# qmoututu11/Image_Restoration_and_Enhancement

Measured on AMD Instinct MI355X. Metric: restored images/sec @512x512, 50 DDIM steps; PSNR/SSIM vs reference, higher is better.
Workload: dtype bf16; 1 GPU; BASELINE configs[1] denoise 512x512, batch 8/GPU, 50 DDIM steps x strength 0.5 = 25 UNet evals, CFG 5.0 (UNet batch 16); task=denoise, global_batch=8, resolution=512, compute=UNet + CLIP bf16, VAE fp16 (fp32 accumulation), parallelism=dp1, weights_bcast=none, outputs_finite=True

## Files before the change

### image_restoration_and_enhancement_amd/_lib.py

```python
from __future__ import annotations

import ctypes as C
import os
from pathlib import Path

_PKG = Path(__file__).resolve().parent
LIB_PATH = Path(os.environ.get("IRX_LIB", _PKG / "libirx.so"))

IRX_F32, IRX_BF16, IRX_F16 = 0, 1, 2
IRX_MODEL_UNET, IRX_MODEL_VAE, IRX_MODEL_CLIP = 0, 1, 2
IRX_MODEL_LPIPS = 3
IRX_MODEL_FID = 4
IRX_MODEL_SRVGG = 5
IRX_LAYOUT_VEC, IRX_LAYOUT_MAT, IRX_LAYOUT_CONV, IRX_LAYOUT_EMB = 0, 1, 2, 3
IRX_LAYOUT_MAT_GEGLU64, IRX_LAYOUT_VEC_GEGLU64 = 4, 5
IRX_LAYOUT_VEC_LN_U, IRX_LAYOUT_VEC_LN_V = 6, 7
IRX_LAYOUT_MAT_CHAIN, IRX_LAYOUT_VEC_CHAIN = 8, 9
IRX_LAYOUT_CONV_UP2 = 10
IRX_RCCL_ID_BYTES = 128
IRX_RESAMPLE_LANCZOS, IRX_RESAMPLE_BICUBIC, IRX_RESAMPLE_MAX_KSIZE = 0, 1, 97


class IrxError(RuntimeError):
    pass
# ... 134 lines not shown
    "irx_op_gn_conv3": (i32, [vp, i32, vp, vp, i32, i32, i32, i32, i32, i32, f32, vp, vp, i32, vp, vp, i32, vp, i64,
                              vp, vp, vp, vp]),
    "irx_op_gn_conv_narrow": (i32, [vp, i32, vp, i32, i32, i32, i32, i32, f32, vp, vp, i32, vp, vp, i32, vp, i32, i32,
                                    vp]),
    "irx_op_gn_proj_ws_bytes": (sz, [i32, i32, i32, i32, i32]),
    "irx_op_gn_proj": (i32, [vp, i32, vp, i32, i32, i32, i32, f32, vp, vp, vp, vp, i32, vp, vp, C.POINTER(i32),
                             C.POINTER(i32)]),
    "irx_op_layer_norm": (i32, [vp, i32, vp, i32, i32, f32, vp, vp, vp]),
    "irx_op_attention": (i32, [vp, i32, i32, i32, i32, i32, i32, vp, i64, i64, vp, i64, i64, vp, i64, i64, vp,
                               i64, i64, f32, i32]),
    "irx_op_attention_hm": (i32, [vp, i32, i32, i32, i32, i32, i32, vp, vp, vp, vp, f32]),
    "irx_op_geglu": (i32, [vp, i32, vp, i32, i32, vp]),
    "irx_op_gemm_geglu": (i32, [vp, i32, i32, i32, i32, vp, vp, vp, vp]),
    "irx_op_gemm_ln_out": (i32, [vp, i32, i32, i32, i32, vp, vp, vp, vp, vp, vp, i32, f32]),
    "irx_op_gemm_ln_fold": (i32, [vp, i32, i32, i32, i32, vp, vp, vp, vp, vp, vp, i32, i32, vp]),
    "irx_op_conv2d_gn_parts": (i32, [vp, i32, vp, vp, i32, i32, i32, i32, i32, i32, i32, vp, vp, i32, i32, i32, i32,
                                     i32, i32, i32, i32, vp, i64, vp, vp, i32, i32, vp, vp, C.POINTER(i32),
                                     C.POINTER(i32), C.POINTER(i32), C.POINTER(sz)]),
    "irx_op_gemm_gn_parts": (i32, [vp, i32, i32, i32, i32, vp, vp, vp, vp, i32, vp, vp, vp, C.POINTER(i32),
                                   C.POINTER(i32), C.POINTER(sz)]),
    "irx_op_upsample_conv_gn_parts": (i32, [vp, i32, vp, i32, i32, i32, i32, vp, vp, vp, vp, vp, C.POINTER(i32),
                                            C.POINTER(i32), C.POINTER(sz)]),
    "irx_op_group_norm_parts": (i32, [vp, i32, vp, vp, i32, i32, i32, i32, i32, f32, vp, vp, i32, vp, vp, i32, vp, i32,
                                      vp]),
    "irx_op_group_norm_parts_ab": (i32, [vp, i32, i32, i32, i32, f32, vp, vp, vp, i32, vp, vp]),
    "irx_op_softmax_rows": (i32, [vp, i32, vp, i64, i32, i32, vp, i64]),
    "irx_op_transpose2d": (i32, [vp, i32, vp, i64, i32, i32, vp, i64, i32, i64, i64]),
    "irx_op_timestep_embed": (i32, [vp, i32, vp, i32, i32, i32, f32, vp]),
    "irx_op_embed_tokens": (i32, [vp, i32, vp, i32, i32, vp, vp, i32, vp]),
}
# ... 89 lines not shown
```

### image_restoration_and_enhancement_amd/csrc/capi.cpp

```cpp
#include <algorithm>
#include <cmath>
#include <cstring>
#include <string>

#include "../../include/irx.h"
#include "gemm_plan.h"
#include "models.h"
#include "profile.h"

namespace irx {
static thread_local std::string g_err;
void set_error(const std::string& m) { g_err = m; }
const char* last_error() { return g_err.c_str(); }
extern int g_attn_pf80;
}

using namespace irx;

struct irx_model {
  std::unique_ptr<Model> m;
};

#define IRX_API_BEGIN try {
#define IRX_API_END                                       \
// ... 971 lines not shown

int irx_op_attention_hm(void* s, int dtype, int B, int H, int lq, int lk, int d, const void* q, const void* k,
                        const void* v, void* o, float scale) {
  IRX_API_BEGIN
  AttnArgs a;
  a.dtype = dtype; a.B = B; a.H = H; a.Lq = lq; a.Lk = lk; a.d = d;
  a.q = q; a.ldq = d; a.sq = (long)H * lq * d; a.hsq = (long)lq * d;
  a.k = k; a.ldk = d; a.sk = (long)H * lk * d; a.hsk = (long)lk * d;
  a.v = v; a.ldv = d; a.sv = (long)H * lk * d; a.hsv = (long)lk * d;
  a.o = o; a.ldo = d; a.so = (long)H * lq * d; a.hso = (long)lq * d;
  a.scale = scale;
  attention(a, S(s));
  IRX_API_END
}

int irx_op_gemm_ln_out(void* s, int dtype, int M, int N, int K, const void* A, const void* B, const float* bias,
                       const void* residual, void* C, void* parts, int final_rs, float eps) {
  IRX_API_BEGIN
  GemmArgs a;
  a.dtype = dtype; a.M = M; a.N = N; a.K = K;
  a.A = A; a.lda = K; a.B = B; a.ldb = K;
  a.C = C; a.ldc = N; a.bias = bias;
  a.residual = residual; a.ldr = N;
  a.imgs = g_op_imgs;
  a.ln_out_rs = final_rs;
  a.ln_eps = eps;
  IRX_CHECK(parts && gemm_emits_ln_parts(a), "shape/dtype cannot emit LayerNorm partials");
  a.ln_out = (float2*)parts;
  gemm(a, S(s));
  IRX_API_END
}

int irx_op_gemm_ln_fold(void* s, int dtype, int M, int N, int K, const void* A, const void* B, const float* u,
                        const float* v, const void* rs, const void* parts, int T, int geglu, void* C) {
  IRX_API_BEGIN
  IRX_CHECK((rs != nullptr) != (parts != nullptr), "give the row statistics or the partials, not both");
  GemmArgs a;
  a.dtype = dtype; a.M = M; a.N = N; a.K = K;
  a.A = A; a.lda = K; a.B = B; a.ldb = K;
  a.C = C; a.ldc = geglu ? N / 2 : N; a.bias = v; a.geglu = geglu ? 1 : 0;
  a.ln_u = u;
  a.ln_rs = (const float2*)rs;
  a.ln_part = (const float2*)parts;
  a.ln_T = parts ? T : 0;
  a.imgs = g_op_imgs;
  IRX_CHECK(!geglu || gemm_geglu_fusable(a), "shape/dtype not eligible for the fused GEGLU epilogue");
  IRX_CHECK(gemm_ln_foldable(a), "shape/dtype not eligible for the folded LayerNorm epilogue");
  gemm(a, S(s));
  IRX_API_END
}

int irx_op_gemm_geglu(void* s, int dtype, int M, int N, int K, const void* A, const void* B, const float* bias,
                      void* C) {
  IRX_API_BEGIN
  GemmArgs a;
  a.dtype = dtype; a.M = M; a.N = N; a.K = K;
  a.A = A; a.lda = K; a.B = B; a.ldb = K;
  a.C = C; a.ldc = N / 2; a.bias = bias; a.geglu = 1;
  a.imgs = g_op_imgs;
// ... 179 lines not shown
```

### image_restoration_and_enhancement_amd/csrc/gemm.hip

```cpp
#include "gemm_plan.h"
#include "profile.h"

namespace irx {

namespace {

constexpr int kThreads = 256;

struct RowInfo {
  int n;
  int iy0, ix0;
};

template <typename T, int WM, int WN, int TM, int TN, bool CONV, bool OUTF32, bool HS = false>
__global__ __launch_bounds__(kThreads, 2) void gemm_kernel(GemmArgs a) {
  constexpr int VEC = 16 / (int)sizeof(T);
  constexpr int BK = 8 * VEC;
  constexpr int BM = WM * TM * 16;
  constexpr int BN = WN * TN * 16;
  constexpr int AR = (BM * 8 + kThreads - 1) / kThreads;
  constexpr int BR = (BN * 8 + kThreads - 1) / kThreads;
  static_assert(WM * WN == 4, "4 waves");
  __shared__ uint4 smem[2][(BM + BN) * 8];

// ... 230 lines not shown
                                a.res_rows < a.M && a.M <= 2 * a.res_rows),
            "repeating residual (res_rows): 16-bit, batch 1, res_rows < M <= 2 res_rows");
  if (a.conv) {
    const ConvGeom& g = a.g;
    IRX_CHECK(g.src0 && g.C0 % vec == 0 && g.C1 % vec == 0, "conv channels must be 16-byte multiples");
    IRX_CHECK(((uintptr_t)g.src0 % 16) == 0 && (!g.src1 || ((uintptr_t)g.src1 % 16) == 0), "conv source alignment");
    IRX_CHECK(g.C1 == 0 || g.src1, "concat source missing");
    IRX_CHECK(a.K == g.KH * g.KW * (g.C0 + g.C1), "conv K mismatch");
    IRX_CHECK(a.M == g.N * g.Ho * g.Wo, "conv M mismatch");
    IRX_CHECK(g.Hv >= g.Hin && g.Wv >= g.Win, "virtual (upsampled) size must not shrink");
  } else {
    IRX_CHECK(a.A && a.lda % vec == 0 && ((uintptr_t)a.A % 16) == 0, "A rows must be 16-byte aligned");
    IRX_CHECK(!a.A1 || (a.batch == 1 && a.kA1 > 0 && a.kA1 < a.K && a.lda1 % vec == 0 && ((uintptr_t)a.A1 % 16) == 0),
              "second A source: batch 1, 0 < kA1 < K, 16-byte rows");
  }
  IRX_CHECK(!a.ln_part || (a.ln_T >= 1 && a.K == a.ln_T * kLnGroup), "LayerNorm partials must cover the K row");
  const GemmPlan p = gemm_plan(a);
  IRX_CHECK(!(a.ln_rs || a.ln_part) || (a.ln_u && p.ln_fold), "folded LayerNorm needs the large-tile path");
  IRX_CHECK(!a.geglu || p.geglu, "GEGLU epilogue needs the large-tile path");
  IRX_CHECK((!a.ln_out || p.ln_out) && (!a.b_rows || p.bimg),
            "LayerNorm partials / per-image weights need the large-tile epilogue");
  IRX_CHECK(!a.gn_part || p.gn_rows > 0, "GroupNorm partials need the large-tile epilogue");
  IRX_CHECK(!a.gn_ab || p.gn_fused, "GroupNorm-fused operand needs the halo conv path");
  IRX_CHECK(!a.A1 || p.path == GEMM_SK || p.large(), "a two-source A (conv1x1_as_dense) needs the large-tile path");
  IRX_CHECK(!a.up2_w || p.up2, "a per-parity upsampler conv (up2) needs the large-tile path");
  switch (p.path) {
    case GEMM_SK:
      IRX_CHECK(gemm_sk(a, s), "gemm_sk declined a call planned for it");
      return;
    case GEMM_HALO:
    case GEMM_LARGE:
// ... 33 lines not shown
```

### image_restoration_and_enhancement_amd/csrc/gemm2.hip

```cpp
#include <cmath>
#include <map>
#include <mutex>
#include <type_traits>
#include <utility>

#include "gemm_plan.h"
#include "profile.h"

namespace irx {

__device__ uint4 g_zero_page[4];
#if defined(IRX_DIAG) || defined(IRX_HALO_STAMPS)
constexpr int kDbgMask = ~0;
#define IRX_HALO_DIAG 1
#else
constexpr int kDbgMask = 0;
#endif
#ifdef IRX_HALO_STAMPS
constexpr int kHaloStampBlocks = 2048;
__device__ unsigned long long g_halo_stamps[kHaloStampBlocks * 8 * 8];
extern "C" int irx_debug_halo_stamps(void* out, int n) {
  if (n > kHaloStampBlocks * 64) n = kHaloStampBlocks * 64;
  return hipMemcpyFromSymbol(out, HIP_SYMBOL(g_halo_stamps), (size_t)n * 8, 0, hipMemcpyDeviceToHost) == hipSuccess ? n : -1;
}
// ... 63 lines not shown
  constexpr int NINST = ROWS / RPI;
  constexpr int IPW = (NINST + NW - 1) / NW;
  constexpr int STAGE = ROWS * CPR;
  constexpr int KSUB = BK / 32;
  static_assert((NW == 8 || NW == 4) && ROWS % RPI == 0 && BM % 16 == 0 && (BK == 32 || BK == 64), "tile shape");
  static_assert(!HALO || (CONV && !RESIZE && S >= 2 && S <= 8 && NW == 8), "halo tiles: 3x3 conv");
  static_assert(!PP || !CONV, "ping-pong: dense GEMMs only");
  constexpr bool STRIP = HALO == 5 || HALO == 7;
  constexpr int NTAP = (HALO == 6 || HALO == 7 || HALO == 9) ? 4 : 9;
  constexpr bool MI = HALO == 8 || HALO == 9;
  constexpr int HB_U4 = (BM + 2 * kHaloWMax) * CPR;
  constexpr int RING = HALO ? 2 * HB_U4 + S * BN * CPR + CPR + 64 : S * STAGE;
  constexpr int RINGX = RING + (!HALO && NINST % NW ? 64 : 0);
  constexpr int SMEM = RINGX > BM * BN / 8 ? RINGX : BM * BN / 8;
  static_assert(SMEM * 16 <= 160 * 1024, "LDS budget");
  __shared__ __attribute__((aligned(16))) uint4 smem[SMEM];

  const int tid = threadIdx.x, lane = tid & 63, wave = tid >> 6;
  const int wm = wave / WN, wn = wave % WN;
  const int tiles_n = a.N / BN + (a.N % BN != 0);
  const int tiles_m = (a.M + BM - 1) / BM;
  const int bid = xcd_remap(blockIdx.x, tiles_m * tiles_n);
  int tile_m, tile_n;
  if (a.group_m > 0) {
    const int gsz = a.group_m * tiles_n, grp = bid / gsz, r = bid - grp * gsz;
    const int gm = min(a.group_m, tiles_m - grp * a.group_m);
    tile_m = grp * a.group_m + r % gm;
    tile_n = r / gm;
  } else {
    tile_n = a.nmajor ? bid / tiles_m : bid % tiles_n;
    tile_m = a.nmajor ? bid % tiles_m : bid / tiles_n;
// ... 127 lines not shown
        const int r = wm * TM * 16 + i * 16 + frow;
        af[i] = As[r * CPR + ((s * 4 + fgrp) ^ swz(r))];
      }
#pragma unroll
      for (int j = 0; j < TN; ++j) {
        const int r = wn * TN * 16 + j * 16 + frow;
        bfr[j] = Bs[r * CPR + ((s * 4 + fgrp) ^ swz(r + BM))];
      }
      if constexpr (S > 2) __builtin_amdgcn_s_setprio(1);
#pragma unroll
      for (int i = 0; i < TM; ++i)
#pragma unroll
        for (int j = 0; j < TN; ++j)
          acc[i][j] = Mfma<T>::m16x16x32(af[i], bfr[j], acc[i][j]);
      if constexpr (S > 2) __builtin_amdgcn_s_setprio(0);
    }
  };

  if constexpr (HALO == 2 || HALO == 4 || HALO >= 5) {
    static_assert(S == 3 && KSUB == 2 && NW == 8 && CPR == 8 && RPI == 8, "ping-pong halo: 3-stage B ring, BK 64");
    constexpr bool DG = HALO == 4;
    const int dbg = DG ? a.dbg : 0;
    const int W = a.g.Win, H = a.g.Hin;
    const int Wl = STRIP ? kStripW : W, lw = __builtin_ctz(Wl);
    const int HW = H * W;
    const int img = m0 / HW;
    int y0 = 0, x0 = 0;
    const int img0 = MI ? m0 >> 6 : 0, nimg = MI ? min(4, (a.M - m0) >> 6) : 0;
    if constexpr (MI) {
    } else if constexpr (STRIP) {
// ... 454 lines not shown
#pragma unroll
      for (int s = 0; s < KSUB; ++s)
#pragma unroll
        for (int i = 0; i < TM; ++i)
#pragma unroll
          for (int j = 0; j < TN; ++j) acc[i][j] = Mfma<T>::m16x16x32(fa[s][i], fb[s][j], acc[i][j]);
    };
    auto barrier = [&](bool drain) {
      __builtin_amdgcn_sched_barrier(0);
      if (drain) asm volatile("s_waitcnt lgkmcnt(0)\n\ts_barrier" ::: "memory");
      else asm volatile("s_barrier" ::: "memory");
      __builtin_amdgcn_sched_barrier(0);
    };
    issueP(kt0, 0);
    issueP(min(kt0 + 1, kt1 - 1), 1);
    wait_vm(IPW);
    barrier(true);
    if (g1) barrier(true);
    for (int kb = kt0; kb < kt1; kb += 3) {
      static_for(std::make_integer_sequence<int, 3>{}, [&](auto uc) {
        constexpr int u = decltype(uc)::value;
        const int kt = kb + u;
        if (kt < kt1) {
          readF(uc);
          issueP(min(kt + 2, kt1 - 1), (u + 2) % 3);
          if (g1) wait_vm(IPW);
          barrier(g1);
          mma();
          if (!g1) wait_vm(IPW);
          barrier(true);
        }
      });
    }
    if (!g1) barrier(true);
    asm volatile("s_waitcnt vmcnt(0)" ::: "memory");
    __syncthreads();
  } else if constexpr (S == 2) {
    if (kt0 < kt1) issue(kt0, 0);
    asm volatile("s_waitcnt vmcnt(0)" ::: "memory");
    __syncthreads();
    for (int kt = kt0; kt < kt1; ++kt) {
      const int st = (kt - kt0) & 1;
      if (kt + 1 < kt1) issue(kt + 1, st ^ 1);
      if (!(a.dbg & kDbgMask & 2)) compute(st);
      asm volatile("s_waitcnt vmcnt(0)" ::: "memory");
      __syncthreads();
    }
  } else {
#pragma unroll
    for (int p = 0; p < S - 1; ++p)
      if (kt0 + p < kt1) issue(kt0 + p, p);
    int st = 0;
    for (int kt = kt0; kt < kt1; ++kt) {
      wait_vm(IPW * min(S - 2, kt1 - 1 - kt));
      asm volatile("s_barrier" ::: "memory");
      if (kt + S - 1 < kt1) issue(kt + S - 1, st == 0 ? S - 1 : st - 1);
      if (!(a.dbg & kDbgMask & 2)) compute(st);
      st = st + 1 == S ? 0 : st + 1;
    }
    asm volatile("s_waitcnt vmcnt(0)" ::: "memory");
    __syncthreads();
  }

  if (a.dbg & kDbgMask & 1) {
    float t = 0.f;
#pragma unroll
// ... 83 lines not shown
      constexpr int kEpiPF = BN <= 128 ? 8 : 6;
      auto csw = [](int c, int row) { return c < (CPR & ~7) ? c ^ (row & 7) : c; };
      if (a.ln_rs || a.ln_part) {
        float uu[TN], bb[TN];
#pragma unroll
        for (int j = 0; j < TN; ++j) {
          const int n = n0 + wn * TN * 16 + j * 16 + frow;
          uu[j] = n < a.N ? a.ln_u[n] : 0.f;
          bb[j] = (biasp && n < a.N) ? biasp[n] : 0.f;
        }
#pragma unroll
        for (int i = 0; i < TM; ++i)
#pragma unroll
          for (int r = 0; r < 4; ++r) {
            const int row = wm * TM * 16 + i * 16 + fgrp * 4 + r;
            const float2 rs = m0 + row < a.M ? ln_rs_at(a.ln_rs, a.ln_part, a.ln_T, a.ln_eps, m0 + row)
                                             : make_float2(0.f, 0.f);
#pragma unroll
            for (int j = 0; j < TN; ++j) {
              const int col = wn * TN * 16 + j * 16 + frow;
              tileS[row * BN + (csw(col >> 3, row) << 3) + (col & 7)] =
                  __builtin_bit_cast(uint16_t, from_f<T>(fmaf(acc[i][j][r], rs.x, fmaf(-rs.y, uu[j], bb[j]))));
            }
          }
      } else {
#pragma unroll
        for (int j = 0; j < TN; ++j) {
          const int col = wn * TN * 16 + j * 16 + frow;
          const float bias = (biasp && n0 + col < a.N) ? biasp[n0 + col] : 0.f;
#pragma unroll
          for (int i = 0; i < TM; ++i)
#pragma unroll
// ... 159 lines not shown
#pragma unroll
          for (int j = 0; j < TPC; ++j) {
            const double2 v = red[col * TPC + j];
            A += v.x;
            B += v.y;
          }
          long rb = m0 / BM;
          if (a.up2_w) {
            const long rpl = (long)a.up2_h * a.up2_w / BM;
            rb = (rb / rpl * 4 + a.up2_p) * rpl + rb % rpl;
          }
          *(double2*)(a.gn_part + (rb * a.N + n0 + col) * 2) = make_double2(A, B);
        }
        return;
      }
      float2* const lno = BN == kLnGroup ? a.ln_out : nullptr;
      if (a.hs_L && !Rp && !a.rowadd && !lno && a.out_scale == 1.f && (a.hs_d & 7) == 0 && a.hs_L % BM == 0 &&
          BN % a.hs_d == 0 && n0 % a.hs_d == 0 && a.hs_C % BN == 0 && m0 + BM <= a.M && n0 + BN <= a.N) {
        const int dch = a.hs_d >> 3, segc = BM * dch;
        const int part = n0 / a.hs_C, hd0 = (n0 - part * a.hs_C) / a.hs_d, heads = a.hs_C / a.hs_d;
        const long img = m0 / a.hs_L, tok0 = m0 - img * a.hs_L;
        uint16_t* const hb = Cp + (long)part * a.M * a.hs_C + ((img * heads + hd0) * a.hs_L + tok0) * a.hs_d;
        const long sstride = (long)a.hs_L * a.hs_d;
        const float inv_segc = 1.f / (float)segc, inv_dch = 1.f / (float)dch;
#pragma unroll 2
        for (int idx = tid; idx < BM * CPR; idx += NT) {
          int seg = (int)((float)idx * inv_segc);
          seg += (seg + 1) * segc <= idx;
          seg -= seg * segc > idx;
          const int rem = idx - seg * segc;
          int row = (int)((float)rem * inv_dch);
// ... 24 lines not shown
            for (int e = 0; e < 8; ++e) f[e] += rv[e];
          }
#pragma unroll
          for (int e = 0; e < 8; ++e) f[e] *= a.out_scale;
          u = Vec16<T>::pack(f);
          if (lno) *ts = u;
        }
        *(uint4*)(Cp + c_off(a, prow(m), n)) = u;
      };
#pragma unroll 1
      for (int idx = tid; idx < BM * CPR; idx += NT) {
        const int row = idx / CPR, c = idx - row * CPR;
        if (m0 + row >= a.M || n0 + c * 8 >= a.N) continue;
        store_chunk(row, c);
      }
      if constexpr (BN == kLnGroup && NT % BM == 0) {
        if (lno) {
          constexpr int G = NT / BM, CPG = CPR / G;
          static_assert(CPR % G == 0 && (G == 1 || G == 2 || G == 4 || G == 8), "LayerNorm partial lanes");
          __syncthreads();
          const int row = tid / G, g = tid % G;
          const uint16_t* trow = tileS + row * BN;
          float x0;
          {
            float f0[8];
            Vec16<T>::unpack(*(const uint4*)(trow + (csw(0, row) << 3)), f0);
            x0 = f0[0];
          }
          float s1 = 0.f, s2 = 0.f;
#pragma unroll 4
          for (int c = g * CPG; c < (g + 1) * CPG; ++c) {
            float f[8];
            Vec16<T>::unpack(*(const uint4*)(trow + (csw(c, row) << 3)), f);
#pragma unroll
            for (int e = 0; e < 8; ++e) {
              const float d = f[e] - x0;
              s1 += d;
              s2 = fmaf(d, d, s2);
            }
          }
#pragma unroll
          for (int o = 1; o < G; o <<= 1) {
            s1 += __shfl_xor(s1, o);
            s2 += __shfl_xor(s2, o);
          }
          const float ds = s1 * (1.f / (float)kLnGroup);
          if (g == 0 && m0 + row < a.M) {
            const float mean = x0 + ds, m2 = fmaxf(fmaf(-s1, ds, s2), 0.f);
            lno[(long)(m0 + row) * (a.N / kLnGroup) + n0 / kLnGroup] =
                a.ln_out_rs ? ln_fin(mean, m2, 1, a.ln_eps) : make_float2(mean, m2);
          }
        }
      }
      return;
    }
  }
#pragma unroll
  for (int i = 0; i < TM; ++i) {
#pragma unroll
    for (int j = 0; j < TN; ++j) {
      const int n = n0 + wn * TN * 16 + j * 16 + frow;
      if (n >= a.N) continue;
      const float bias = biasp ? biasp[n] : 0.f;
#pragma unroll
      for (int r = 0; r < 4; ++r) {
// ... 284 lines not shown
```

### image_restoration_and_enhancement_amd/csrc/gemm_plan.cpp

```cpp
#include "gemm_plan.h"

#include <algorithm>
#include <cmath>

namespace irx {

bool g_large_tiles = true;
int g_large_mask = 3;
int g_large_dense = 63;
int g_small_splitk = 1;
int g_gemm_sk = 1;
int g_gemm_deep = 0;
bool g_gemm_small = false;
int g_gemm_small_kmax = 1280;
int g_gemm_force = 0;
bool g_tile_256x320 = true;
bool g_splitk_inkernel = true;
int g_gemm_nmajor = 1;
int g_gemm_group = 1;
int g_gemm_pp = 2;
int g_gemm_pp2 = 1;
int g_gemm_pp_chain = 1;
int g_conv1x1_dense = 1;
int g_conv_halo = 1;
// ... 376 lines not shown
  if (a.gn_ab) p.gn_fused = g_gn_fuse && p.path == GEMM_HALO && p.HALO == 1;
  if (a.gn_part && g_gn_parts && p.large() && vec && one16 && !a.geglu && !a.hs_L) {
    if (p.splits > 1 && !p.inkernel)
      p.gn_rows = (g_gn_red_parts && !a.up2_w && !a.b_rows && a.M % kRedGnRows == 0 && a.N % 64 == 0 && a.act == ACT_NONE)
                      ? kRedGnRows : 0;
    else if (p.path == GEMM_HALO)
      p.gn_rows = h.mode == 3 ? 0 : 256;
    else if (a.up2_w && ((long)a.up2_h * a.up2_w) % p.BM)
      p.gn_rows = 0;
    else
      p.gn_rows = a.M % p.BM ? 0 : p.BM;
  }
  if (a.ln_rs || a.ln_part)
    p.ln_fold = !a.conv && a.alpha == 1.f && one16 && vec_ok(a) && (p.path == GEMM_SK || (p.path == GEMM_LARGE && full_epi));
  const bool staged = p.path == GEMM_LARGE && full_epi && !a.conv && one16 && !a.geglu && g_gemm_deep == 0;
  if (a.ln_out && g_ln_parts && staged && !a.hs_L && !a.gn_part && a.N % kLnGroup == 0 && !(a.ln_out_rs && a.N != kLnGroup)) {
    GemmArgs bare = a;
    bare.ln_out = nullptr;
    p.ln_out = p.BN == kLnGroup && (p.BM == 256 || p.BM == 128) && !gemm_sk_eligible(bare);
  }
  if (a.b_rows > 0)
    p.bimg = staged && !(p.WM == 2 && p.WN == 2) && a.M % a.b_rows == 0 && a.b_rows % p.BM == 0;
  return p;
}

size_t gemm_workspace_bytes(const GemmArgs& a) { return gemm_plan(a).ws_reserve; }

size_t gemm_small_split_bytes(const GemmArgs& a) {
  const int sp = small_splits(a);
  return sp ? (size_t)sp * a.M * a.N * sizeof(float) : 0;
}

int gemm_large_splits(const GemmArgs& a) {
  const GemmPlan p = gemm_plan(a);
// ... 49 lines not shown
```

### image_restoration_and_enhancement_amd/csrc/models.cpp

```cpp
#include "models.h"

#include <cmath>
#include <cstdio>
#include <vector>

namespace irx {

static size_t align_up(size_t x, size_t a) { return (x + a - 1) / a * a; }

int g_arena_guard = 0;
int g_ff_chain = 1;
int g_up2 = 1;
constexpr size_t kGuard = 64 * 1024;

void* Arena::alloc(size_t bytes) {
  bytes = align_up(bytes ? bytes : 1, 256) + (g_arena_guard ? kGuard : 0);
  size_t off = (size_t)-1;
  for (auto it = free_.begin(); it != free_.end(); ++it) {
    if (it->second >= bytes) {
      off = it->first;
      const size_t rest = it->second - bytes;
      free_.erase(it);
      if (rest) free_[off + bytes] = rest;
      break;
// ... 402 lines not shown
  Act sc;
  const void* res = x0.p;
  if (r.shortcut) {
    sc = new_act(c, B, H, W, r.cout);
    conv2d(c, x0, x1, r.scw, r.scb, r.cout, 1, 1, 0, 0, H, W, sc);
    res = sc.p;
  }
  Act out = new_act(c, B, H, W, r.cout);
  gn_conv3(c, h1, nullptr, r.n2w, r.n2b, eps, 1, r.c2w, r.c2b, r.cout, out, nullptr, 0, res, true);
  drop(c, h1);
  if (r.shortcut) drop(c, sc);
  return out;
}

void Unet::ln_gemm(Ctx& c, GemmArgs& g, const void* x, int rows, int C, P lnw, P lnb, P u, P v, const float* bias,
                   void* nbuf, float2* st, const float2* parts) {
  g.lda = C;
  if (!ln_fold_) {
    lnorm(c, x, rows, C, lnw, lnb, 1e-5f, nbuf);
    g.A = nbuf;
    g.bias = bias;
  } else {
    g.bias = fptr(v);
    g.A = x;
    g.ln_u = fptr(u);
    g.ln_rs = parts ? parts : st;
    if (gemm_ln_foldable(g)) {
      if (!parts && !c.ws->dry()) layer_norm_stats(dt_, x, C, rows, C, 1e-5f, st, c.s);
    } else {
      g.ln_rs = nullptr;
      g.ln_part = nullptr;
      g.ln_u = nullptr;
      if (!c.ws->dry()) layer_norm(dt_, x, C, rows, C, 1e-5f, nullptr, nullptr, nbuf, C, c.s);
      g.A = nbuf;
    }
  }
  run_gemm(c, g);
}

const float2* Unet::xf_proj(Ctx& c, const void* A, int M, int C, P w, const float* bias, void* out,
                            const void* residual, int imgs, float2* lnp, long res_rows) {
  GemmArgs a;
  a.dtype = dt_;
  a.M = M; a.N = C; a.K = C;
  a.A = A; a.lda = C;
  a.B = ptr(w); a.ldb = C;
  a.C = out; a.ldc = C;
  a.bias = bias;
  a.residual = residual; a.ldr = C; a.res_rows = res_rows;
  a.imgs = imgs;
  a.ln_out_rs = 1;
  a.ln_eps = 1e-5f;
  const bool emit = lnp && gemm_emits_ln_parts(a);
  if (emit) a.ln_out = lnp;
  run_gemm(c, a);
  return emit ? lnp : nullptr;
}

Act Unet::transformer(Ctx& c, const XfW& a, Act& x, const void* kv, int L, bool dup) {
  const int B = x.n, HW = x.h * x.w, C = a.c;
  const long M = (long)B * HW;
  const int Bo = dup ? 2 * B : B;
  const long Mo = dup ? 2 * M : M;
  const size_t es = dsize(dt_);
  const int heads = cfg_.heads, d = C / heads;
  const float scale = 1.0f / std::sqrt((float)d);
  Act h = new_act(c, B, x.h, x.w, C);
  float2* lnp = (ln_fold_ && C == kLnGroup) ? (float2*)c.ws->alloc(Mo * sizeof(float2)) : nullptr;
  const float2* parts = nullptr;
  GemmArgs pg;
  pg.dtype = dt_; pg.M = M; pg.N = C; pg.K = C;
  pg.A = x.p; pg.lda = C; pg.ldb = C;
  pg.C = h.p; pg.ldc = C;
  pg.imgs = B;
  pg.b_rows = HW; pg.b_img_stride = (long)C * C; pg.bias_img_stride = C;
  pg.B = ptr(a.piw);
  if (dt_ != F32 && g_gn_fold && C <= 320 && x.gnp && HW % x.gnr == 0 && gemm_bimg_ok(pg)) {
    float2* ab = (float2*)c.ws->alloc((size_t)B * C * sizeof(float2));
    void* wf = c.ws->alloc((size_t)B * C * C * es);
    float* bf = (float*)c.ws->alloc((size_t)B * C * sizeof(float));
    float2* mr = (float2*)c.ws->alloc((size_t)B * cfg_.norm_groups * sizeof(float2));
    if (!c.ws->dry()) {
      group_norm_parts_ab(C, B, HW, cfg_.norm_groups, 1e-6f, fptr(a.nw), fptr(a.nb), x.gnp, x.gnr, ab, mr, c.s);
      gn_fold_weights(dt_, ptr(a.piw), fptr(a.pib), ab, fptr(a.nb), mr, cfg_.norm_groups, C, C, B, wf, bf, c.s);
    }
    pg.B = wf;
    pg.bias = bf;
    pg.ln_out_rs = 1;
    pg.ln_eps = 1e-5f;
    if (lnp && gemm_emits_ln_parts(pg)) {
      pg.ln_out = lnp;
      parts = lnp;
    }
    run_gemm(c, pg);
    c.ws->free(mr);
    c.ws->free(bf);
    c.ws->free(wf);
    c.ws->free(ab);
  } else {
    Act gn = new_act(c, B, x.h, x.w, C);
    gnorm(c, x, nullptr, a.nw, a.nb, 1e-6f, 0, gn);
    parts = xf_proj(c, gn.p, M, C, a.piw, fptr(a.pib), h.p, nullptr, B, lnp);
    drop(c, gn);
  }
  void* n = c.ws->alloc(Mo * C * es);
  void* att = c.ws->alloc(M * C * es);
  float2* st = ln_fold_ ? (float2*)c.ws->alloc(Mo * sizeof(float2)) : nullptr;
// ... 606 lines not shown
```

### image_restoration_and_enhancement_amd/csrc/models.h

```cpp
#pragma once
#include <map>
#include <memory>
#include <vector>

#include "../../include/irx.h"
#include "ops.h"

namespace irx {

extern int g_vae_attn_rows;
extern int g_vae_flash;

class Arena {
 public:
  void reset(char* base, size_t cap) {
    base_ = base; cap_ = cap; end_ = 0; peak_ = 0; free_.clear(); live_.clear(); ids_.clear(); next_id_ = 0;
  }
  void* alloc(size_t bytes);
  void free(void* p);
  size_t peak() const { return peak_; }
  bool dry() const { return base_ == nullptr; }

 private:
  char* base_ = nullptr;
// ... 78 lines not shown
  int kind_;
  irx_model_config cfg_;
  int dt_;
  std::vector<ParamEntry> params_;
  size_t blob_bytes_ = 0;
  char* blob_ = nullptr;
};

struct ResW {
  P n1w, n1b, c1w, c1b, n2w, n2b, c2w, c2b, scw, scb;
  int cin = 0, cout = 0;
  bool shortcut = false;
  long temb_off = -1;
};

class Unet : public Model {
 public:
  Unet(const irx_model_config& cfg, int dtype);
  int cin_pad() const { return cin_pad_; }
  size_t workspace_bytes(int B, int h, int w, int cfg_share = 0, const float* time_proj = nullptr);
  long temb_cols() const { return temb_cols_; }
  size_t time_table_ws(int n);
  void time_table(hipStream_t s, const float* t, int n, float* table, char* ws, size_t cap);
  size_t context_bytes(int B, int L) const { return (size_t)B * L * kv_cols_ * dsize(dt_); }
  void prepare_context(hipStream_t s, const void* ctx, int B, int L, void* kv, char* ws, size_t cap);
  void forward(hipStream_t s, const void* x, int B, int h, int w, const float* t, const void* kv, int L, float* eps,
               char* ws, size_t cap, int cfg_share = 0, const float* time_proj = nullptr);

 private:
  struct XfW {
// ... 8 lines not shown
    std::vector<ResW> res;
    std::vector<XfW> attn;
    bool has_attn = false, resample = false;
    P rsw, rsb;
    P rsw2;
    int ch = 0;
  };
  ResW make_res(const std::string& p, int cin, int cout);
  XfW make_xf(const std::string& p, int c);
  void run(Ctx& c, const void* x, int B, int h, int w, const float* t, const void* kv, int L, float* eps,
           int cfg_share, const float* time_proj);
  void time_chain(Ctx& c, const float* t, int n, float* tproj);
  Act resnet(Ctx& c, const ResW& r, Act& x0, Act* x1, const float* tproj, long tld, float eps);
  Act transformer(Ctx& c, const XfW& a, Act& x, const void* kv, int L, bool dup = false);
  void ln_gemm(Ctx& c, GemmArgs& g, const void* x, int rows, int C, P lnw, P lnb, P u, P v, const float* bias,
               void* nbuf, float2* st, const float2* parts = nullptr);
  const float2* xf_proj(Ctx& c, const void* A, int M, int C, P w, const float* bias, void* out, const void* residual,
                        int imgs, float2* lnp, long res_rows = 0);

  int cin_pad_ = 8;
  bool ln_fold_ = false;
  int temb_dim_ = 1280;
  long temb_cols_ = 0, kv_cols_ = 0;
  std::vector<std::string> temb_names_w_, temb_names_b_, kv_names_;
  P conv_in_w, conv_in_b, t1w, t1b, t2w, t2b, tpw, tpb, kvw, nout_w, nout_b, conv_out_w, conv_out_b;
  std::vector<Block> down_, up_;
  ResW mid_res0_, mid_res1_;
  XfW mid_attn_;
};

class Vae : public Model {
 public:
  Vae(const irx_model_config& cfg, int dtype);
// ... 90 lines not shown
```

### image_restoration_and_enhancement_amd/csrc/ops.h

```cpp
#pragma once
#include "irx_common.h"

namespace irx {

struct ConvGeom {
  const void* src0 = nullptr;
  const void* src1 = nullptr;
  int C0 = 0, C1 = 0;
  int N = 0, Hin = 0, Win = 0;
  int Hv = 0, Wv = 0;
  int KH = 1, KW = 1, stride = 1, pad_t = 0, pad_l = 0;
  int Ho = 0, Wo = 0;
};

struct GemmArgs {
  int dtype = BF16;
  int M = 0, N = 0, K = 0;
  int conv = 0;
  ConvGeom g;
  const void* A = nullptr; long lda = 0; long sA = 0;
  const void* A1 = nullptr; long lda1 = 0; int kA1 = 0;
  const void* B = nullptr; long ldb = 0; long sB = 0;
  void* C = nullptr; long ldc = 0; long sC = 0;
  int out_f32 = 0;
// ... 1 lines not shown
  const float* bias = nullptr;
  const float* rowadd = nullptr; long rowadd_ld = 0; int rows_per_group = 1;
  const void* residual = nullptr; long ldr = 0; long sR = 0;
  long res_rows = 0;
  float out_scale = 1.f;
  int act = ACT_NONE;
  int batch = 1;
  int imgs = 0;
  int vec_epilogue = 0;
  int geglu = 0;
  int hs_L = 0, hs_C = 0, hs_d = 0;
  const float2* gn_ab = nullptr; int gn_silu = 0;
  double* gn_part = nullptr;
  const float2* ln_rs = nullptr; const float* ln_u = nullptr;
  const float2* ln_part = nullptr; int ln_T = 0; float ln_eps = 1e-5f;
  float2* ln_out = nullptr;
  int ln_out_rs = 0;
  int b_rows = 0; long b_img_stride = 0; long bias_img_stride = 0;
  int up2_h = 0, up2_w = 0, up2_p = 0;
  void* splitk_ws = nullptr; size_t splitk_ws_bytes = 0;
  int nmajor = 0;
  int group_m = 0;
  int dbg = 0;
};
constexpr int kCanonImages = 16;
constexpr int kLnGroup = 320;
__device__ __forceinline__ float2 ln_fin(float mean, float m2, int T, float eps) {
  const float inv_n = T == 1 ? 1.f / 320.f : T == 2 ? 1.f / 640.f : 1.f / (float)(T * kLnGroup);
  const float rstd = rsqrtf(fmaf(m2, inv_n, eps));
  return make_float2(rstd, rstd * mean);
}
__device__ __forceinline__ float2 ln_merge(const float2* __restrict__ p, int T) {
  if (T == 1) return p[0];
  if (T == 2) {
    const float2 x = p[0], y = p[1];
    const float d = x.x - y.x;
    return make_float2((x.x + y.x) * 0.5f, fmaf(0.5f * (float)kLnGroup * d, d, x.y + y.y));
  }
  float sm = 0.f;
  for (int t = 0; t < T; ++t) sm += p[t].x;
  const float mean = sm * (1.f / (float)T);
  float m2 = 0.f;
  for (int t = 0; t < T; ++t) {
    const float2 v = p[t];
    const float d = v.x - mean;
    m2 += fmaf((float)kLnGroup * d, d, v.y);
  }
  return make_float2(mean, m2);
}
__device__ __forceinline__ float2 ln_rs_at(const float2* __restrict__ rs, const float2* __restrict__ part, int T,
                                           float eps, long m) {
  if (!part) return rs[m];
  const float2 v = ln_merge(part + m * T, T);
  return ln_fin(v.x, v.y, T, eps);
}
__host__ __device__ __forceinline__ long c_off_f(long m, int n, long ldc, int M, int hs_L, int hs_C, int hs_d, int up2_w,
                                                 int up2_p) {
  if (up2_w) return (2 * (m + (long)up2_w * (m / up2_w)) + 2L * up2_w * (up2_p >> 1) + (up2_p & 1)) * ldc + n;
  if (hs_L == 0) return m * ldc + n;
  const int part = n / hs_C, rem = n - part * hs_C, hd = rem / hs_d, e = rem - hd * hs_d;
  const long img = m / hs_L, tok = m - img * hs_L;
  return (long)part * M * hs_C + ((img * (hs_C / hs_d) + hd) * hs_L + tok) * hs_d + e;
}
#define c_off(a, m, n) c_off_f((m), (n), (a).ldc, (a).M, (a).hs_L, (a).hs_C, (a).hs_d, (a).up2_w, (a).up2_p)
void gemm(const GemmArgs& a, hipStream_t s);
bool gemm_sk(const GemmArgs& a, hipStream_t s);
bool gemm_sk_eligible(const GemmArgs& a);
float* splitk_scratch(size_t bytes);
void splitk_reduce(const GemmArgs& a, const float* ws, int splits, int Mp, int Np, int batch, hipStream_t s);
// ... 198 lines not shown
```

### include/irx.h

```cpp
#ifndef IRX_H_
#define IRX_H_
#include <stddef.h>
#include <stdint.h>

#ifdef __cplusplus
extern "C" {
#endif

#define IRX_F32 0
#define IRX_BF16 1
#define IRX_F16 2

#define IRX_MODEL_UNET 0
#define IRX_MODEL_VAE 1
#define IRX_MODEL_CLIP 2
#define IRX_MODEL_LPIPS 3
#define IRX_MODEL_FID 4
#define IRX_MODEL_SRVGG 5

#define IRX_LAYOUT_VEC 0
#define IRX_LAYOUT_MAT 1
#define IRX_LAYOUT_CONV 2
#define IRX_LAYOUT_EMB 3
#define IRX_LAYOUT_MAT_GEGLU64 4
// ... 217 lines not shown
                   void* ws, int* folded, int* splits);
int irx_op_layer_norm(void* stream, int dtype, const void* x, int rows, int c, float eps, const float* gamma,
                      const float* beta, void* out);
int irx_op_attention(void* stream, int dtype, int batch, int heads, int lq, int lk, int d, const void* q, long ldq,
                     long sq, const void* k, long ldk, long sk, const void* v, long ldv, long sv, void* o, long ldo,
                     long so, float scale, int causal);
int irx_op_attention_hm(void* stream, int dtype, int batch, int heads, int lq, int lk, int d, const void* q,
                        const void* k, const void* v, void* o, float scale);
int irx_op_geglu(void* stream, int dtype, const void* proj, int M, int F, void* out);
int irx_op_gemm_geglu(void* stream, int dtype, int M, int N, int K, const void* A, const void* B, const float* bias,
                      void* C);
int irx_op_gemm_ln_out(void* stream, int dtype, int M, int N, int K, const void* A, const void* B, const float* bias,
                       const void* residual, void* C, void* parts, int final_rs, float eps);
int irx_op_gemm_ln_fold(void* stream, int dtype, int M, int N, int K, const void* A, const void* B, const float* u,
                        const float* v, const void* rs, const void* parts, int T, int geglu, void* C);
int irx_op_conv2d_gn_parts(void* stream, int dtype, const void* x0, const void* x1, int c0, int c1, int n, int hin,
                           int win, int hv, int wv, const void* weight, const float* bias, int cout, int kh, int kw,
                           int stride, int pad_t, int pad_l, int ho, int wo, const float* rowadd, long rowadd_ld,
                           const void* residual, void* out, int out_f32, int act, double* parts, void* ws, int* rows,
                           int* splits, int* halo, size_t* ws_bytes);
int irx_op_gemm_gn_parts(void* stream, int dtype, int M, int N, int K, const void* A, const void* B, const float* bias,
                         const void* residual, int imgs, void* C, double* parts, void* ws, int* rows, int* splits,
                         size_t* ws_bytes);
int irx_op_upsample_conv_gn_parts(void* stream, int dtype, const void* x, int n, int h, int w, int c, const void* w2,
                                  const float* bias, void* out, double* parts, void* ws, int* up2_ok, int* rows,
                                  size_t* ws_bytes);
int irx_op_group_norm_parts(void* stream, int dtype, const void* x0, const void* x1, int c0, int c1, int n, int hw,
                            int groups, float eps, const float* gamma, const float* beta, int silu, void* out,
                            const double* p0, int r0, const double* p1, int r1, void* ws);
int irx_op_group_norm_parts_ab(void* stream, int c0, int n, int hw, int groups, float eps, const float* gamma,
// ... 14 lines not shown
```

Baseline: 18.30 images/s.

## Emit LayerNorm partials over 128-column groups for wide transformer channels

Extends the GEMM LayerNorm-partials epilogue so it can emit per-row mean/M2 partials over 128-column tiles as well as 320. Transformer blocks with 640/1280 channels can then skip the standalone layer_norm_stats pass and fold LayerNorm into the next GEMM, merging the partials instead. It also caches per-row LN stats in an LDS table once per block rather than recomputing them per fragment in the epilogue. The wide path is gated on g_ln_parts >= 2 and on tile constraints (BM 128, 8 waves). Merging adds a little work per row, and the extra LDS can lower occupancy.

```diff
diff --git a/image_restoration_and_enhancement_amd/_lib.py b/image_restoration_and_enhancement_amd/_lib.py
--- a/image_restoration_and_enhancement_amd/_lib.py
+++ b/image_restoration_and_enhancement_amd/_lib.py
@@ -172,6 +172,8 @@
     "irx_op_gemm_geglu": (i32, [vp, i32, i32, i32, i32, vp, vp, vp, vp]),
     "irx_op_gemm_ln_out": (i32, [vp, i32, i32, i32, i32, vp, vp, vp, vp, vp, vp, i32, f32]),
     "irx_op_gemm_ln_fold": (i32, [vp, i32, i32, i32, i32, vp, vp, vp, vp, vp, vp, i32, i32, vp]),
+    "irx_op_gemm_ln_out_w": (i32, [vp, i32, i32, i32, i32, vp, vp, vp, vp, i64, vp, vp, i32, i32, f32]),
+    "irx_op_gemm_ln_fold_w": (i32, [vp, i32, i32, i32, i32, vp, vp, vp, vp, vp, vp, i32, i32, i32, vp]),
     "irx_op_conv2d_gn_parts": (i32, [vp, i32, vp, vp, i32, i32, i32, i32, i32, i32, i32, vp, vp, i32, i32, i32, i32,
                                      i32, i32, i32, i32, vp, i64, vp, vp, i32, i32, vp, vp, C.POINTER(i32),
                                      C.POINTER(i32), C.POINTER(i32), C.POINTER(sz)]),
diff --git a/image_restoration_and_enhancement_amd/csrc/capi.cpp b/image_restoration_and_enhancement_amd/csrc/capi.cpp
--- a/image_restoration_and_enhancement_amd/csrc/capi.cpp
+++ b/image_restoration_and_enhancement_amd/csrc/capi.cpp
@@ -1009,16 +1009,20 @@
   IRX_API_END
 }
 
-int irx_op_gemm_ln_out(void* s, int dtype, int M, int N, int K, const void* A, const void* B, const float* bias,
-                       const void* residual, void* C, void* parts, int final_rs, float eps) {
-  IRX_API_BEGIN
+int irx_op_gemm_ln_out_w(void* s, int dtype, int M, int N, int K, const void* A, const void* B, const float* bias,
+                         const void* residual, long res_rows, void* C, void* parts, int width, int final_rs,
+                         float eps) {
+  IRX_API_BEGIN
+  IRX_CHECK(width == kLnGroup || width == kLnGroupNarrow, "LayerNorm partials span 320 or 128 columns");
+  IRX_CHECK(!res_rows || (residual && res_rows > 0 && M <= 2 * res_rows), "res_rows: a residual, M <= 2 res_rows");
   GemmArgs a;
   a.dtype = dtype; a.M = M; a.N = N; a.K = K;
   a.A = A; a.lda = K; a.B = B; a.ldb = K;
   a.C = C; a.ldc = N; a.bias = bias;
-  a.residual = residual; a.ldr = N;
+  a.residual = residual; a.ldr = N; a.res_rows = res_rows;
   a.imgs = g_op_imgs;
   a.ln_out_rs = final_rs;
+  a.ln_W = width;
   a.ln_eps = eps;
   IRX_CHECK(parts && gemm_emits_ln_parts(a), "shape/dtype cannot emit LayerNorm partials");
   a.ln_out = (float2*)parts;
@@ -1026,10 +1030,21 @@
   IRX_API_END
 }
 
+int irx_op_gemm_ln_out(void* s, int dtype, int M, int N, int K, const void* A, const void* B, const float* bias,
+                       const void* residual, void* C, void* parts, int final_rs, float eps) {
+  return irx_op_gemm_ln_out_w(s, dtype, M, N, K, A, B, bias, residual, 0, C, parts, kLnGroup, final_rs, eps);
+}
+
 int irx_op_gemm_ln_fold(void* s, int dtype, int M, int N, int K, const void* A, const void* B, const float* u,
                         const float* v, const void* rs, const void* parts, int T, int geglu, void* C) {
+  return irx_op_gemm_ln_fold_w(s, dtype, M, N, K, A, B, u, v, rs, parts, T, kLnGroup, geglu, C);
+}
+
+int irx_op_gemm_ln_fold_w(void* s, int dtype, int M, int N, int K, const void* A, const void* B, const float* u,
+                          const float* v, const void* rs, const void* parts, int T, int width, int geglu, void* C) {
   IRX_API_BEGIN
   IRX_CHECK((rs != nullptr) != (parts != nullptr), "give the row statistics or the partials, not both");
+  IRX_CHECK(width == kLnGroup || width == kLnGroupNarrow, "LayerNorm partials span 320 or 128 columns");
   GemmArgs a;
   a.dtype = dtype; a.M = M; a.N = N; a.K = K;
   a.A = A; a.lda = K; a.B = B; a.ldb = K;
@@ -1038,6 +1053,7 @@
   a.ln_rs = (const float2*)rs;
   a.ln_part = (const float2*)parts;
   a.ln_T = parts ? T : 0;
+  a.ln_W = width;
   a.imgs = g_op_imgs;
   IRX_CHECK(!geglu || gemm_geglu_fusable(a), "shape/dtype not eligible for the fused GEGLU epilogue");
   IRX_CHECK(gemm_ln_foldable(a), "shape/dtype not eligible for the folded LayerNorm epilogue");
diff --git a/image_restoration_and_enhancement_amd/csrc/gemm.hip b/image_restoration_and_enhancement_amd/csrc/gemm.hip
--- a/image_restoration_and_enhancement_amd/csrc/gemm.hip
+++ b/image_restoration_and_enhancement_amd/csrc/gemm.hip
@@ -268,7 +268,9 @@
     IRX_CHECK(!a.A1 || (a.batch == 1 && a.kA1 > 0 && a.kA1 < a.K && a.lda1 % vec == 0 && ((uintptr_t)a.A1 % 16) == 0),
               "second A source: batch 1, 0 < kA1 < K, 16-byte rows");
   }
-  IRX_CHECK(!a.ln_part || (a.ln_T >= 1 && a.K == a.ln_T * kLnGroup), "LayerNorm partials must cover the K row");
+  IRX_CHECK(!(a.ln_part || a.ln_out) || a.ln_W == kLnGroup || a.ln_W == kLnGroupNarrow,
+            "LayerNorm partials span 320 or 128 columns");
+  IRX_CHECK(!a.ln_part || (a.ln_T >= 1 && a.K == a.ln_T * a.ln_W), "LayerNorm partials must cover the K row");
   const GemmPlan p = gemm_plan(a);
   IRX_CHECK(!(a.ln_rs || a.ln_part) || (a.ln_u && p.ln_fold), "folded LayerNorm needs the large-tile path");
   IRX_CHECK(!a.geglu || p.geglu, "GEGLU epilogue needs the large-tile path");
diff --git a/image_restoration_and_enhancement_amd/csrc/gemm2.hip b/image_restoration_and_enhancement_amd/csrc/gemm2.hip
--- a/image_restoration_and_enhancement_amd/csrc/gemm2.hip
+++ b/image_restoration_and_enhancement_amd/csrc/gemm2.hip
@@ -101,7 +101,11 @@
   constexpr int RINGX = RING + (!HALO && NINST % NW ? 64 : 0);
   constexpr int SMEM = RINGX > BM * BN / 8 ? RINGX : BM * BN / 8;
   static_assert(SMEM * 16 <= 160 * 1024, "LDS budget");
-  __shared__ __attribute__((aligned(16))) uint4 smem[SMEM];
+  constexpr bool LNTAB = !CONV && !OUTF32 && HALO == 0 && SMEM * 16 + BM * 8 <= 160 * 1024;
+  constexpr int LNT_U4 = LNTAB ? BM / 2 : 0;
+  static_assert(!LNTAB || NT >= BM, "one thread per table row");
+  __shared__ __attribute__((aligned(16))) uint4 smem[SMEM + LNT_U4];
+  float2* const lnT = (float2*)(smem + SMEM);
 
   const int tid = threadIdx.x, lane = tid & 63, wave = tid >> 6;
   const int wm = wave / WN, wn = wave % WN;
@@ -259,6 +263,15 @@
         for (int j = 0; j < TN; ++j)
           acc[i][j] = Mfma<T>::m16x16x32(af[i], bfr[j], acc[i][j]);
       if constexpr (S > 2) __builtin_amdgcn_s_setprio(0);
+    }
+  };
+
+  auto ln_table = [&]() {
+    if constexpr (LNTAB) {
+      if ((a.ln_rs || a.ln_part) && tid < BM) {
+        const long m = m0 + tid;
+        lnT[tid] = m < a.M ? ln_rs_at(a.ln_rs, a.ln_part, a.ln_T, a.ln_eps, m, a.ln_W) : make_float2(0.f, 0.f);
+      }
     }
   };
 
@@ -743,6 +756,7 @@
     };
     issueP(kt0, 0);
     issueP(min(kt0 + 1, kt1 - 1), 1);
+    ln_table();
     wait_vm(IPW);
     barrier(true);
     if (g1) barrier(true);
@@ -766,6 +780,7 @@
     __syncthreads();
   } else if constexpr (S == 2) {
     if (kt0 < kt1) issue(kt0, 0);
+    ln_table();
     asm volatile("s_waitcnt vmcnt(0)" ::: "memory");
     __syncthreads();
     for (int kt = kt0; kt < kt1; ++kt) {
@@ -779,6 +794,7 @@
 #pragma unroll
     for (int p = 0; p < S - 1; ++p)
       if (kt0 + p < kt1) issue(kt0 + p, p);
+    ln_table();
     int st = 0;
     for (int kt = kt0; kt < kt1; ++kt) {
       wait_vm(IPW * min(S - 2, kt1 - 1 - kt));
@@ -892,8 +908,10 @@
 #pragma unroll
           for (int r = 0; r < 4; ++r) {
             const int row = wm * TM * 16 + i * 16 + fgrp * 4 + r;
-            const float2 rs = m0 + row < a.M ? ln_rs_at(a.ln_rs, a.ln_part, a.ln_T, a.ln_eps, m0 + row)
-                                             : make_float2(0.f, 0.f);
+            float2 rs;
+            if constexpr (LNTAB) rs = lnT[row];
+            else rs = m0 + row < a.M ? ln_rs_at(a.ln_rs, a.ln_part, a.ln_T, a.ln_eps, m0 + row, a.ln_W)
+                                     : make_float2(0.f, 0.f);
 #pragma unroll
             for (int j = 0; j < TN; ++j) {
               const int col = wn * TN * 16 + j * 16 + frow;
@@ -1083,7 +1101,9 @@
         }
         return;
       }
-      float2* const lno = BN == kLnGroup ? a.ln_out : nullptr;
+      constexpr bool LNOUT = (BN == kLnGroup && NT % BM == 0) ||
+                             (BN == kLnGroupNarrow && BM == 128 && NW == 8 && !CONV && !PP && HALO == 0);
+      float2* const lno = LNOUT ? a.ln_out : nullptr;
       if (a.hs_L && !Rp && !a.rowadd && !lno && a.out_scale == 1.f && (a.hs_d & 7) == 0 && a.hs_L % BM == 0 &&
           BN % a.hs_d == 0 && n0 % a.hs_d == 0 && a.hs_C % BN == 0 && m0 + BM <= a.M && n0 + BN <= a.N) {
         const int dch = a.hs_d >> 3, segc = BM * dch;
@@ -1138,7 +1158,7 @@
         if (m0 + row >= a.M || n0 + c * 8 >= a.N) continue;
         store_chunk(row, c);
       }
-      if constexpr (BN == kLnGroup && NT % BM == 0) {
+      if constexpr (LNOUT) {
         if (lno) {
           constexpr int G = NT / BM, CPG = CPR / G;
           static_assert(CPR % G == 0 && (G == 1 || G == 2 || G == 4 || G == 8), "LayerNorm partial lanes");
@@ -1168,11 +1188,11 @@
             s1 += __shfl_xor(s1, o);
             s2 += __shfl_xor(s2, o);
           }
-          const float ds = s1 * (1.f / (float)kLnGroup);
+          const float ds = s1 * (1.f / (float)BN);
           if (g == 0 && m0 + row < a.M) {
             const float mean = x0 + ds, m2 = fmaxf(fmaf(-s1, ds, s2), 0.f);
-            lno[(long)(m0 + row) * (a.N / kLnGroup) + n0 / kLnGroup] =
-                a.ln_out_rs ? ln_fin(mean, m2, 1, a.ln_eps) : make_float2(mean, m2);
+            lno[(long)(m0 + row) * (a.N / BN) + n0 / BN] =
+                a.ln_out_rs ? ln_fin(mean, m2, 1, a.ln_eps, BN) : make_float2(mean, m2);
           }
         }
       }
diff --git a/image_restoration_and_enhancement_amd/csrc/gemm_plan.cpp b/image_restoration_and_enhancement_amd/csrc/gemm_plan.cpp
--- a/image_restoration_and_enhancement_amd/csrc/gemm_plan.cpp
+++ b/image_restoration_and_enhancement_amd/csrc/gemm_plan.cpp
@@ -414,10 +414,14 @@
   if (a.ln_rs || a.ln_part)
     p.ln_fold = !a.conv && a.alpha == 1.f && one16 && vec_ok(a) && (p.path == GEMM_SK || (p.path == GEMM_LARGE && full_epi));
   const bool staged = p.path == GEMM_LARGE && full_epi && !a.conv && one16 && !a.geglu && g_gemm_deep == 0;
-  if (a.ln_out && g_ln_parts && staged && !a.hs_L && !a.gn_part && a.N % kLnGroup == 0 && !(a.ln_out_rs && a.N != kLnGroup)) {
+  const bool ln_w_ok = a.ln_W == kLnGroup || a.ln_W == kLnGroupNarrow;
+  if (a.ln_out && g_ln_parts && staged && !a.hs_L && !a.gn_part && ln_w_ok && a.N % a.ln_W == 0 &&
+      !(a.ln_out_rs && a.N != a.ln_W)) {
     GemmArgs bare = a;
     bare.ln_out = nullptr;
-    p.ln_out = p.BN == kLnGroup && (p.BM == 256 || p.BM == 128) && !gemm_sk_eligible(bare);
+    const bool tile = a.ln_W == kLnGroup ? (p.BM == 256 || p.BM == 128)
+                                         : (p.BM == 128 && p.WM * p.WN == 8 && !p.PP);
+    p.ln_out = p.BN == a.ln_W && tile && !gemm_sk_eligible(bare);
   }
   if (a.b_rows > 0)
     p.bimg = staged && !(p.WM == 2 && p.WN == 2) && a.M % a.b_rows == 0 && a.b_rows % p.BM == 0;
diff --git a/image_restoration_and_enhancement_amd/csrc/models.cpp b/image_restoration_and_enhancement_amd/csrc/models.cpp
--- a/image_restoration_and_enhancement_amd/csrc/models.cpp
+++ b/image_restoration_and_enhancement_amd/csrc/models.cpp
@@ -440,7 +440,7 @@
 }
 
 void Unet::ln_gemm(Ctx& c, GemmArgs& g, const void* x, int rows, int C, P lnw, P lnb, P u, P v, const float* bias,
-                   void* nbuf, float2* st, const float2* parts) {
+                   void* nbuf, float2* st, LnStats parts) {
   g.lda = C;
   if (!ln_fold_) {
     lnorm(c, x, rows, C, lnw, lnb, 1e-5f, nbuf);
@@ -450,9 +450,10 @@
     g.bias = fptr(v);
     g.A = x;
     g.ln_u = fptr(u);
-    g.ln_rs = parts ? parts : st;
+    if (parts.p && parts.T > 0) { g.ln_part = parts.p; g.ln_T = parts.T; g.ln_W = parts.W; }
+    else g.ln_rs = parts.p ? parts.p : st;
     if (gemm_ln_foldable(g)) {
-      if (!parts && !c.ws->dry()) layer_norm_stats(dt_, x, C, rows, C, 1e-5f, st, c.s);
+      if (!parts.p && !c.ws->dry()) layer_norm_stats(dt_, x, C, rows, C, 1e-5f, st, c.s);
     } else {
       g.ln_rs = nullptr;
       g.ln_part = nullptr;
@@ -464,7 +465,7 @@
   run_gemm(c, g);
 }
 
-const float2* Unet::xf_proj(Ctx& c, const void* A, int M, int C, P w, const float* bias, void* out,
+LnStats Unet::xf_proj(Ctx& c, const void* A, int M, int C, P w, const float* bias, void* out,
                             const void* residual, int imgs, float2* lnp, long res_rows) {
   GemmArgs a;
   a.dtype = dt_;
@@ -475,12 +476,25 @@
   a.bias = bias;
   a.residual = residual; a.ldr = C; a.res_rows = res_rows;
   a.imgs = imgs;
-  a.ln_out_rs = 1;
   a.ln_eps = 1e-5f;
-  const bool emit = lnp && gemm_emits_ln_parts(a);
-  if (emit) a.ln_out = lnp;
+  LnStats st;
+  if (lnp && C == kLnGroup) {
+    a.ln_out_rs = 1;
+    if (gemm_emits_ln_parts(a)) st.p = lnp;
+  } else if (lnp) {
+    for (int W : {kLnGroup, kLnGroupNarrow}) {
+      if (C % W) continue;
+      a.ln_W = W;
+      if (gemm_emits_ln_parts(a)) {
+        st.p = lnp; st.T = C / W; st.W = W;
+        break;
+      }
+    }
+  }
+  if (st.p) a.ln_out = lnp;
+  else { a.ln_out_rs = 0; a.ln_W = kLnGroup; }
   run_gemm(c, a);
-  return emit ? lnp : nullptr;
+  return st;
 }
 
 Act Unet::transformer(Ctx& c, const XfW& a, Act& x, const void* kv, int L, bool dup) {
@@ -492,8 +506,11 @@
   const int heads = cfg_.heads, d = C / heads;
   const float scale = 1.0f / std::sqrt((float)d);
   Act h = new_act(c, B, x.h, x.w, C);
-  float2* lnp = (ln_fold_ && C == kLnGroup) ? (float2*)c.ws->alloc(Mo * sizeof(float2)) : nullptr;
-  const float2* parts = nullptr;
+  const bool ln_wide = ln_fold_ && g_ln_parts >= 2 && C != kLnGroup && C % kLnGroupNarrow == 0;
+  float2* lnp = (ln_fold_ && C == kLnGroup) ? (float2*)c.ws->alloc(Mo * sizeof(float2))
+                : ln_wide                   ? (float2*)c.ws->alloc(Mo * (C / kLnGroupNarrow) * sizeof(float2))
+                                            : nullptr;
+  LnStats parts;
   GemmArgs pg;
   pg.dtype = dt_; pg.M = M; pg.N = C; pg.K = C;
   pg.A = x.p; pg.lda = C; pg.ldb = C;
@@ -516,7 +533,7 @@
     pg.ln_eps = 1e-5f;
     if (lnp && gemm_emits_ln_parts(pg)) {
       pg.ln_out = lnp;
-      parts = lnp;
+      parts.p = lnp;
     }
     run_gemm(c, pg);
     c.ws->free(mr);
diff --git a/image_restoration_and_enhancement_amd/csrc/models.h b/image_restoration_and_enhancement_amd/csrc/models.h
--- a/image_restoration_and_enhancement_amd/csrc/models.h
+++ b/image_restoration_and_enhancement_amd/csrc/models.h
@@ -116,6 +116,8 @@
   long temb_off = -1;
 };
 
+struct LnStats { const float2* p = nullptr; int T = 0; int W = 0; };
+
 class Unet : public Model {
  public:
   Unet(const irx_model_config& cfg, int dtype);
@@ -154,9 +156,9 @@
   Act resnet(Ctx& c, const ResW& r, Act& x0, Act* x1, const float* tproj, long tld, float eps);
   Act transformer(Ctx& c, const XfW& a, Act& x, const void* kv, int L, bool dup = false);
   void ln_gemm(Ctx& c, GemmArgs& g, const void* x, int rows, int C, P lnw, P lnb, P u, P v, const float* bias,
-               void* nbuf, float2* st, const float2* parts = nullptr);
-  const float2* xf_proj(Ctx& c, const void* A, int M, int C, P w, const float* bias, void* out, const void* residual,
-                        int imgs, float2* lnp, long res_rows = 0);
+               void* nbuf, float2* st, LnStats parts = LnStats());
+  LnStats xf_proj(Ctx& c, const void* A, int M, int C, P w, const float* bias, void* out, const void* residual,
+                  int imgs, float2* lnp, long res_rows = 0);
 
   int cin_pad_ = 8;
   bool ln_fold_ = false;
diff --git a/image_restoration_and_enhancement_amd/csrc/ops.h b/image_restoration_and_enhancement_amd/csrc/ops.h
--- a/image_restoration_and_enhancement_amd/csrc/ops.h
+++ b/image_restoration_and_enhancement_amd/csrc/ops.h
@@ -39,6 +39,7 @@
   double* gn_part = nullptr;
   const float2* ln_rs = nullptr; const float* ln_u = nullptr;
   const float2* ln_part = nullptr; int ln_T = 0; float ln_eps = 1e-5f;
+  int ln_W = 320;
   float2* ln_out = nullptr;
   int ln_out_rs = 0;
   int b_rows = 0; long b_img_stride = 0; long bias_img_stride = 0;
@@ -50,17 +51,18 @@
 };
 constexpr int kCanonImages = 16;
 constexpr int kLnGroup = 320;
-__device__ __forceinline__ float2 ln_fin(float mean, float m2, int T, float eps) {
-  const float inv_n = T == 1 ? 1.f / 320.f : T == 2 ? 1.f / 640.f : 1.f / (float)(T * kLnGroup);
+constexpr int kLnGroupNarrow = 128;
+__device__ __forceinline__ float2 ln_fin(float mean, float m2, int T, float eps, int W = kLnGroup) {
+  const float inv_n = W == kLnGroup && T == 1 ? 1.f / 320.f : W == kLnGroup && T == 2 ? 1.f / 640.f : 1.f / (float)(T * W);
   const float rstd = rsqrtf(fmaf(m2, inv_n, eps));
   return make_float2(rstd, rstd * mean);
 }
-__device__ __forceinline__ float2 ln_merge(const float2* __restrict__ p, int T) {
+__device__ __forceinline__ float2 ln_merge(const float2* __restrict__ p, int T, int W = kLnGroup) {
   if (T == 1) return p[0];
   if (T == 2) {
     const float2 x = p[0], y = p[1];
     const float d = x.x - y.x;
-    return make_float2((x.x + y.x) * 0.5f, fmaf(0.5f * (float)kLnGroup * d, d, x.y + y.y));
+    return make_float2((x.x + y.x) * 0.5f, fmaf(0.5f * (float)W * d, d, x.y + y.y));
   }
   float sm = 0.f;
   for (int t = 0; t < T; ++t) sm += p[t].x;
@@ -69,15 +71,15 @@
   for (int t = 0; t < T; ++t) {
     const float2 v = p[t];
     const float d = v.x - mean;
-    m2 += fmaf((float)kLnGroup * d, d, v.y);
+    m2 += fmaf((float)W * d, d, v.y);
   }
   return make_float2(mean, m2);
 }
 __device__ __forceinline__ float2 ln_rs_at(const float2* __restrict__ rs, const float2* __restrict__ part, int T,
-                                           float eps, long m) {
+                                           float eps, long m, int W = kLnGroup) {
   if (!part) return rs[m];
-  const float2 v = ln_merge(part + m * T, T);
-  return ln_fin(v.x, v.y, T, eps);
+  const float2 v = ln_merge(part + m * T, T, W);
+  return ln_fin(v.x, v.y, T, eps, W);
 }
 __host__ __device__ __forceinline__ long c_off_f(long m, int n, long ldc, int M, int hs_L, int hs_C, int hs_d, int up2_w,
                                                  int up2_p) {
diff --git a/include/irx.h b/include/irx.h
--- a/include/irx.h
+++ b/include/irx.h
@@ -255,6 +255,11 @@
                        const void* residual, void* C, void* parts, int final_rs, float eps);
 int irx_op_gemm_ln_fold(void* stream, int dtype, int M, int N, int K, const void* A, const void* B, const float* u,
                         const float* v, const void* rs, const void* parts, int T, int geglu, void* C);
+int irx_op_gemm_ln_out_w(void* stream, int dtype, int M, int N, int K, const void* A, const void* B, const float* bias,
+                         const void* residual, long res_rows, void* C, void* parts, int width, int final_rs,
+                         float eps);
+int irx_op_gemm_ln_fold_w(void* stream, int dtype, int M, int N, int K, const void* A, const void* B, const float* u,
+                          const float* v, const void* rs, const void* parts, int T, int width, int geglu, void* C);
 int irx_op_conv2d_gn_parts(void* stream, int dtype, const void* x0, const void* x1, int c0, int c1, int n, int hin,
                            int win, int hv, int wv, const void* weight, const float* bias, int cout, int kh, int kw,
                            int stride, int pad_t, int pad_l, int ho, int wo, const float* rowadd, long rowadd_ld,
```

Result: faster. 18.51 images/s (median of 6 runs) (+1.2%).
